# ChengZhang-98/lqer

Measured on AMD Instinct MI355X. Metric: W4A8+rank-r Linear GEMM TFLOPS-equiv, higher is better.
Workload: dtype bf16; 1 GPU; LqerLinear 4096x4096 rank32 W4A8-MXINT16 M=2048 (BASELINE configs[1]); rank=32, formats=x MXINT8/16, W MXINT4/16, A_out,B_out as x, y fp16, weights=one Linear

## Files before the change

include/lqer_hip.h:

```cpp
#ifndef LQER_HIP_H
#define LQER_HIP_H

#include <stddef.h>
#include <stdint.h>

#ifdef __cplusplus
extern "C" {
#endif

#define LQER_ABI_VERSION 14

#define LQER_OK 0
#define LQER_E_INVALID (-1)
#define LQER_E_UNSUPPORTED (-2)
#define LQER_E_LAUNCH (-3)
#define LQER_E_WORKSPACE (-4)

#define LQER_F32 0
#define LQER_F16 1
#define LQER_BF16 2

#define LQER_Q_PASSTHROUGH 0
#define LQER_Q_MXINT 1
#define LQER_Q_PASSTHROUGH_F16 2

#define LQER_Q_MXINT_I8 3

#define LQER_Q_INT 4

#define LQER_Q_MINIFLOAT 5

#define LQER_K_ALIGN 64
#define LQER_M_ALIGN 256
#define LQER_N_ALIGN 256
#define LQER_R_ALIGN 16
#define LQER_PANEL_ROWS 16
#define LQER_PANEL_BYTES 576

typedef struct lqer_qfmt {
  int32_t kind;
  int32_t width;
  int32_t block;
  int32_t exp_width;
  int32_t exp_bias;
} lqer_qfmt_t;

typedef struct lqer_linear_desc {
  int32_t in_features;
  int32_t out_features;
  int32_t rank;
  int32_t has_bias;
  lqer_qfmt_t x_fmt;
  lqer_qfmt_t w_fmt;
  lqer_qfmt_t b_fmt;
  lqer_qfmt_t a_out_fmt;
  lqer_qfmt_t b_out_fmt;
  int32_t tuning;
} lqer_linear_desc_t;

#define LQER_TUNE_TILE_ROWS_128 0x1
#define LQER_TUNE_TILE_ROWS_64 0x2
#define LQER_TUNE_I8_ROWS_128 0x4
#define LQER_TUNE_I8_ROWS_256 0x8
#define LQER_TUNE_AMAX_ATOMIC 0x40000
#define LQER_TUNE_AMAX_PARTS 0x80000
#define LQER_TUNE_AMAX_XCH_MISS 0x100000
#define LQER_TUNE_ACT8_SPLIT 0x200000
#define LQER_TUNE_ACT8_FUSED 0x400000
#define LQER_TUNE_ACT16_SPLIT 0x800000
#define LQER_TUNE_ACT16_FUSED 0x1000000
#define LQER_TUNE_AMAX_NO_MRX 0x4000000
#define LQER_TUNE_BOUT_IN_PROLOGUE 0x2000000
#define LQER_TUNE_DECODE_NO_POLL 0x10000

typedef struct lqer_linear_sizes {
  size_t w_packed;
  size_t a_t;
  size_t b_t;
  size_t bias_q;
  size_t workspace;
} lqer_linear_sizes_t;

int lqer_version(void);
const char* lqer_last_error(void);
size_t lqer_sizeof_qfmt(void);
size_t lqer_sizeof_linear_desc(void);
size_t lqer_sizeof_linear_sizes(void);
size_t lqer_sizeof_group_member(void);

int64_t lqer_padded_k(int64_t K);
int64_t lqer_padded_n(int64_t N);
int64_t lqer_padded_m(int64_t M);
int64_t lqer_padded_r(int64_t r);


int lqer_quantize_mxint(const void* x, int dtype, int64_t rows, int64_t cols, int64_t ld,
                        const lqer_qfmt_t* fmt, float* deq_f32, int8_t* codes, int8_t* exps,
                        void* stream);

int lqer_quantize_mxint_tiles(const void* x, int dtype, int64_t batches, int64_t rows, int64_t cols, const lqer_qfmt_t* fmt,
                              int64_t tile_rows, int64_t tile_cols, float* deq_f32, float* amax_scratch, void* stream);

int lqer_quantize_act_mxint(const void* x, int dtype, int64_t M, int64_t K, int64_t ldx,
                            const lqer_qfmt_t* fmt, void* xq_bf16, void* stream);


int lqer_linear_sizes(const lqer_linear_desc_t* desc, int64_t m_max, lqer_linear_sizes_t* out);

int lqer_pack_weight_mxint(const void* W, int dtype, int64_t N, int64_t K, int64_t ldw,
                           const lqer_qfmt_t* fmt, void* w_packed, void* scratch, void* stream);
int lqer_pack_weight_mxint_2d(const void* W, int dtype, int64_t N, int64_t K, int64_t ldw,
                              const lqer_qfmt_t* fmt, int64_t block_rows, void* w_packed, void* scratch,
                              void* stream);

int lqer_unpack_weight_mxint(const void* w_packed, int64_t N, int64_t K, const lqer_qfmt_t* fmt,
                             float* w_f32, void* stream);

int lqer_pack_lowrank(const void* A, const void* B, int dtype, int64_t K, int64_t N, int64_t r,
                      void* a_t, void* b_t, int32_t* limb_flags, void* stream);

int lqer_pack_bias(const void* bias, int dtype, int64_t N, const lqer_qfmt_t* fmt, float* bias_q,
                   void* stream);


int lqer_linear_forward(const lqer_linear_desc_t* desc, const void* x, int dtype, int64_t M,
                        int64_t ldx, const void* w_packed, const void* a_t, const void* b_t,
                        int a_limbs, int b_limbs, const float* bias_q, void* y, int64_t ldy,
                        void* workspace, size_t workspace_bytes, void* stream);


int lqer_quantize_act_xa(const lqer_linear_desc_t* desc, const void* x, int dtype, int64_t M,
                         int64_t ldx, const void* a_t, int a_limbs, void* xq_bf16, void* xaq_bf16,
                         void* scratch, size_t scratch_bytes, void* stream);
size_t lqer_lowrank_xa_scratch_bytes(const lqer_linear_desc_t* desc, int64_t m_max);
size_t lqer_act_image_bytes(const lqer_linear_desc_t* desc, int64_t m_max);
int lqer_lowrank_xa(const lqer_linear_desc_t* desc, const void* xq_bf16, int64_t M,
                    const void* a_t, int a_limbs, void* xaq_bf16, void* scratch,
                    size_t scratch_bytes, void* stream);
size_t lqer_linear_gemm_scratch_bytes(const lqer_linear_desc_t* desc, int64_t m_max);
int lqer_linear_gemm(const lqer_linear_desc_t* desc, const void* xq_bf16, int64_t M,
                     const void* w_packed, const void* xaq_bf16, const void* b_t, int b_limbs,
                     const float* bias_q, void* y, int dtype, int64_t ldy, void* scratch,
                     size_t scratch_bytes, void* stream);
int lqer_quantize_act_xa_prep(const lqer_linear_desc_t* desc, const void* x, int dtype, int64_t M,
                              int64_t ldx, const void* a_t, int a_limbs, void* xq_bf16, void* xaq_bf16,
                              void* scratch, size_t scratch_bytes, void* gemm_scratch, size_t* ready_bytes, void* stream);
int lqer_linear_gemm_prepared(const lqer_linear_desc_t* desc, const void* xq_bf16, int64_t M,
                              const void* w_packed, const void* xaq_bf16, const void* b_t, int b_limbs,
                              const float* bias_q, void* y, int dtype, int64_t ldy, void* scratch,
                              size_t scratch_bytes, size_t ready_bytes, void* stream);

#define LQER_ROUTE_SMALLM 0
#define LQER_ROUTE_TILE128 1
#define LQER_ROUTE_TILE256 2
#define LQER_ROUTE_I8 3
// ... 64 lines not shown
```

lqer_amd/_lib.py:

```python
from __future__ import annotations

import ctypes as C
import os
import subprocess
from typing import Optional

_HERE = os.path.dirname(os.path.abspath(__file__))
LIB_PATH = os.environ.get("LQER_AMD_LIB") or os.path.join(_HERE, "liblqer_hip.so")
BUILD_SCRIPT = os.path.join(_HERE, "csrc", "build.sh")

ABI_VERSION = 14
F32, F16, BF16 = 0, 1, 2
Q_PASSTHROUGH, Q_MXINT, Q_PASSTHROUGH_F16, Q_MXINT_I8, Q_INT, Q_MINIFLOAT = 0, 1, 2, 3, 4, 5
K_ALIGN, M_ALIGN, N_ALIGN, R_ALIGN = 64, 256, 256, 16
ROUTE_SMALLM, ROUTE_TILE128, ROUTE_TILE256, ROUTE_I8 = 0, 1, 2, 3
TUNE_TILE_ROWS_128, TUNE_TILE_ROWS_64, TUNE_DECODE_NO_POLL = 0x1, 0x2, 0x10000
TUNE_I8_ROWS_128, TUNE_I8_ROWS_256, TUNE_AMAX_ATOMIC, TUNE_AMAX_PARTS = 0x4, 0x8, 0x40000, 0x80000
TUNE_ACT16_SPLIT, TUNE_ACT16_FUSED = 0x800000, 0x1000000
TUNE_ACT8_SPLIT, TUNE_ACT8_FUSED = 0x200000, 0x400000
TUNE_AMAX_NO_MRX = 0x4000000
TUNE_BOUT_IN_PROLOGUE = 0x2000000
TUNE_AMAX_XCH_MISS = 0x100000


class QFmt(C.Structure):
    _fields_ = [("kind", C.c_int32), ("width", C.c_int32), ("block", C.c_int32), ("exp_width", C.c_int32), ("exp_bias", C.c_int32)]


class LinearDesc(C.Structure):
    _fields_ = [
        ("in_features", C.c_int32),
        ("out_features", C.c_int32),
        ("rank", C.c_int32),
        ("has_bias", C.c_int32),
        ("x_fmt", QFmt),
        ("w_fmt", QFmt),
        ("b_fmt", QFmt),
        ("a_out_fmt", QFmt),
        ("b_out_fmt", QFmt),
        ("tuning", C.c_int32),
    ]


class GroupMember(C.Structure):
    _fields_ = [("desc", C.POINTER(LinearDesc)), ("w_packed", C.c_void_p), ("b_t", C.c_void_p), ("b_limbs", C.c_int32),
                ("bias_q", C.c_void_p), ("y", C.c_void_p), ("ldy", C.c_int64)]


class LinearSizes(C.Structure):
    _fields_ = [("w_packed", C.c_size_t), ("a_t", C.c_size_t), ("b_t", C.c_size_t), ("bias_q", C.c_size_t), ("workspace", C.c_size_t)]


_vp, _i, _i64, _sz = C.c_void_p, C.c_int, C.c_int64, C.c_size_t
_qp, _dp = C.POINTER(QFmt), C.POINTER(LinearDesc)
_sp = C.POINTER(C.c_int64)

SIGNATURES = {
    "lqer_version": (_i, []),
    "lqer_last_error": (C.c_char_p, []),
    "lqer_sizeof_qfmt": (_sz, []),
    "lqer_sizeof_linear_desc": (_sz, []),
    "lqer_sizeof_linear_sizes": (_sz, []),
    "lqer_sizeof_group_member": (_sz, []),
    "lqer_padded_k": (_i64, [_i64]),
    "lqer_padded_n": (_i64, [_i64]),
    "lqer_padded_m": (_i64, [_i64]),
    "lqer_padded_r": (_i64, [_i64]),
    "lqer_quantize_mxint": (_i, [_vp, _i, _i64, _i64, _i64, _qp, _vp, _vp, _vp, _vp]),
    "lqer_quantize_mxint_tiles": (_i, [_vp, _i, _i64, _i64, _i64, _qp, _i64, _i64, _vp, _vp, _vp]),
    "lqer_quantize_act_mxint": (_i, [_vp, _i, _i64, _i64, _i64, _qp, _vp, _vp]),
    "lqer_linear_sizes": (_i, [_dp, _i64, C.POINTER(LinearSizes)]),
    "lqer_pack_weight_mxint": (_i, [_vp, _i, _i64, _i64, _i64, _qp, _vp, _vp, _vp]),
    "lqer_pack_weight_mxint_2d": (_i, [_vp, _i, _i64, _i64, _i64, _qp, _i64, _vp, _vp, _vp]),
    "lqer_unpack_weight_mxint": (_i, [_vp, _i64, _i64, _qp, _vp, _vp]),
    "lqer_pack_lowrank": (_i, [_vp, _vp, _i, _i64, _i64, _i64, _vp, _vp, _vp, _vp]),
    "lqer_pack_bias": (_i, [_vp, _i, _i64, _qp, _vp, _vp]),
    "lqer_linear_forward": (_i, [_dp, _vp, _i, _i64, _i64, _vp, _vp, _vp, _i, _i, _vp, _vp, _i64, _vp, _sz, _vp]),
    "lqer_quantize_act_xa": (_i, [_dp, _vp, _i, _i64, _i64, _vp, _i, _vp, _vp, _vp, _sz, _vp]),
    "lqer_lowrank_xa_scratch_bytes": (_sz, [_dp, _i64]),
    "lqer_act_image_bytes": (_sz, [_dp, _i64]),
    "lqer_lowrank_xa": (_i, [_dp, _vp, _i64, _vp, _i, _vp, _vp, _sz, _vp]),
    "lqer_linear_gemm_scratch_bytes": (_sz, [_dp, _i64]),
    "lqer_linear_gemm": (_i, [_dp, _vp, _i64, _vp, _vp, _vp, _i, _vp, _vp, _i, _i64, _vp, _sz, _vp]),
    "lqer_quantize_act_xa_prep": (_i, [_dp, _vp, _i, _i64, _i64, _vp, _i, _vp, _vp, _vp, _sz, _vp, C.POINTER(_sz), _vp]),
    "lqer_linear_gemm_prepared": (_i, [_dp, _vp, _i64, _vp, _vp, _vp, _i, _vp, _vp, _i, _i64, _vp, _sz, _sz, _vp]),
    "lqer_linear_gemm_ld": (_i, [_dp, _vp, _i64, _vp, _vp, _i64, _vp, _i, _vp, _vp, _i, _i64, _vp, _sz, _vp]),
    "lqer_desc_limbs": (_i, [_dp, C.POINTER(C.c_int), C.POINTER(C.c_int)]),
    "lqer_replicate_rows": (_i, [_vp, _vp, _i64, _i64, _i, _vp]),
    "lqer_decode_partials": (_i, [_dp, _i64]),
    "lqer_tile_partials": (_i, [_dp, _i64, _i]),
    "lqer_group_workspace_bytes": (_sz, [_i64, _i64]),
    "lqer_linear_forward_group": (_i, [C.POINTER(GroupMember), _i, _vp, _i, _i64, _i64, _vp, _i, _vp, _sz, _vp]),
    "lqer_gemm_route": (_i, [_dp, _i64, _i]),
    "lqer_gemm_tile_rows": (_i, [_dp, _i64, _i]),
    "lqer_f16_prepare": (_i, [_vp, _i64, _i64, _vp, _i, _i64, _vp, _vp, _vp]),
    "lqer_a_f16_image_bytes": (C.c_size_t, [_i64, _i64]),
    "lqer_a_b16_image_bytes": (C.c_size_t, [_i64, _i64]),
    "lqer_a_b16_prepare": (_i, [_vp, _i64, _i64, _vp, _vp]),
    "lqer_i8_prepare": (_i, [_vp, _i64, _i64, _qp, _vp, _vp]),
    "lqer_unpack_weight_i8": (_i, [_vp, _i64, _i64, _vp, _vp]),
    "lqer_unpack_weight_i8_fmt": (_i, [_vp, _i64, _i64, _qp, _vp, _vp]),
    "lqer_quantize_act_i8": (_i, [_vp, _i, _i64, _i64, _i64, _qp, _vp, _vp]),
    "lqer_clock_probe": (_i, [_vp, _i, _i64, _vp]),
    "lqer_col_abs_stats_workspace_bytes": (_sz, [_i64, _i64]),
# ... 47 lines not shown
```

lqer_amd/csrc/gemm_w4a8.hip:

```cpp
#include <atomic>
#include <type_traits>

#include "common.h"

namespace lqer {

constexpr int BM = 128, BN = 256, BK = 64;
#ifndef LQER_DEPTH
#define LQER_DEPTH 3
#endif
constexpr int DEPTH = LQER_DEPTH;
constexpr int NSLOT = DEPTH + 1;
constexpr int R_SLOT = (BN / 16) * LQER_PANEL_BYTES;
constexpr int OFF_A = 0;
constexpr int a_slot_bytes(int mt) { return 32 * mt * BK * 2; }
constexpr int gemm_lds_bytes(int mt) { return NSLOT * a_slot_bytes(mt) + NSLOT * R_SLOT; }

__device__ __forceinline__ int swz(int r, int c) { return r * 128 + ((c ^ ((r >> 1) & 7)) << 4); }

typedef __attribute__((address_space(3))) void lds_void;
typedef __attribute__((address_space(1))) const void gbl_void;

__device__ __forceinline__ float pair32_max(float v) {
  auto r = __builtin_amdgcn_permlane32_swap(__float_as_uint(v), __float_as_uint(v), false, false);
  return fmaxf(__uint_as_float(r[0]), __uint_as_float(r[1]));
}


template <int OFF>
__device__ __forceinline__ bf16x8 lds_read128(uint32_t addr) {
  bf16x8 v;
  asm volatile("ds_read_b128 %0, %1 offset:%2" : "=v"(v) : "v"(addr), "i"(OFF));
  return v;
}
__device__ __forceinline__ u32x4 lds_read128u(uint32_t addr) {
  u32x4 v;
  asm volatile("ds_read_b128 %0, %1" : "=v"(v) : "v"(addr));
  return v;
}
__device__ __forceinline__ uint32_t lds_read32_512(uint32_t addr) {
  uint32_t v;
  asm volatile("ds_read_b32 %0, %1 offset:512" : "=v"(v) : "v"(addr));
  return v;
}
__device__ __forceinline__ u32x2 lds_read64(uint32_t addr) {
  u32x2 v;
  asm volatile("ds_read_b64 %0, %1" : "=v"(v) : "v"(addr));
  return v;
}
__device__ __forceinline__ int lds_read_i8_512(uint32_t addr) {
  int v;
  asm volatile("ds_read_i8 %0, %1 offset:512" : "=v"(v) : "v"(addr));
  return v;
}
__device__ __forceinline__ void lds_write128(uint32_t addr, u32x4 v) {
  asm volatile("ds_write_b128 %0, %1" ::"v"(addr), "v"(v) : "memory");
}
__device__ __forceinline__ void lds_wait(bf16x8& a, bf16x8& b, bf16x8& c, bf16x8& d) {
  asm volatile("s_waitcnt lgkmcnt(0)" : "+v"(a), "+v"(b), "+v"(c), "+v"(d));
}
__device__ __forceinline__ void lds_wait(bf16x8& a, bf16x8& b) {
  asm volatile("s_waitcnt lgkmcnt(0)" : "+v"(a), "+v"(b));
}
__device__ __forceinline__ void lds_wait(u32x2& a, int& b) {
  asm volatile("s_waitcnt lgkmcnt(0)" : "+v"(a), "+v"(b));
}

#ifdef LQER_STAMPS
#define LQER_LOAD_BARRIER ""
#else
#define LQER_LOAD_BARRIER "\n\ts_barrier"
#endif
#if defined(LQER_STAMPS) || defined(LQER_CLOCKPROBE)
__device__ unsigned long long* g_stamp_buf = nullptr;
#endif
#ifdef LQER_STAMPS
#define STAMP(i)                                                                        \
  do {                                                                                  \
    unsigned long long t_;                                                              \
    __builtin_amdgcn_sched_barrier(0);                                                  \
    asm volatile("s_memtime %0\n\ts_waitcnt lgkmcnt(0)" : "=s"(t_)::"memory");         \
    __builtin_amdgcn_sched_barrier(0);                                                  \
    st_sum[i] += t_ - st_prev;                                                          \
    st_prev = t_;                                                                       \
  } while (0)
#else
#define STAMP(i)
#endif

template <int DT, bool LOWRANK, int BOUT, bool STAGED = false, int MT = 4, bool WTWOS = false, bool DEFER = false, bool WMF = false>
__global__ __launch_bounds__(512) void k_lqer_gemm(GemmArgs g) {
  static_assert(MT == 4 || MT == 2, "128- or 64-row tiles");
  static_assert(!DEFER || (LOWRANK && BOUT == 1 && MT == 4), "deferred B_out: blocks of 16 on 128-row tiles");
  static_assert(!WTWOS || DT != LQER_F16X, "integer weights: no fp16 main loop");
  constexpr int BMk = 32 * MT;
  constexpr int AP = MT / 2;
  constexpr bool XF16 = DT == LQER_F16X;
  constexpr int A_SLOT = a_slot_bytes(MT), OFF_R = NSLOT * A_SLOT;
  extern __shared__ __attribute__((aligned(16))) unsigned char smem[];
  const int tid = threadIdx.x, lane = tid & 63;
  const int wave = __builtin_amdgcn_readfirstlane(tid >> 6);
  const int wn = wave;
  const int l31 = lane & 31, lh = lane >> 5;
#ifdef LQER_CLOCKPROBE
  unsigned long long cp_rin, cp_rq = 0;
  asm volatile("s_memrealtime %0\n\ts_waitcnt lgkmcnt(0)" : "=s"(cp_rin)::"memory");
#endif

  const int nt = g.tiles_m * g.tiles_n;
  int tile;
  {
    const int b = blockIdx.x, xcd = b & 7, q8 = nt >> 3, r8 = nt & 7;
    tile = (xcd < r8 ? xcd * (q8 + 1) : r8 * (q8 + 1) + (xcd - r8) * q8) + (b >> 3);
  }
  const int tm = tile / g.tiles_n, tn = tile - tm * g.tiles_n;
  const int m0 = tm * BMk, n0 = tn * BN;
  const int nk = g.Kp / BK;

  const auto a_rsrc = __builtin_amdgcn_make_buffer_rsrc((void*)(g.xq + (int64_t)m0 * g.Kp), 0, BMk * g.Kp * 2, 0x00020000);
  int a_voff[2] = {0, 0};
#pragma unroll
  for (int i = 0; i < AP; ++i) {
    const int row = wave * (8 * AP) + i * 8 + (lane >> 3);
    const int chunk = (lane & 7) ^ ((row >> 1) & 7);
    a_voff[i] = (row * g.Kp + chunk * 8) * 2;
  }
  const uint8_t* w_base = g.wp + ((int64_t)(n0 / 16) * nk) * LQER_PANEL_BYTES;
  const auto w_rsrc = __builtin_amdgcn_make_buffer_rsrc((void*)w_base, 0, 16 * nk * LQER_PANEL_BYTES, 0x00020000);
  auto w_piece_voff = [&](int piece) {
    const int byte = piece * 1024 + lane * 16;
    const int pnl = byte / LQER_PANEL_BYTES;
    return pnl * nk * LQER_PANEL_BYTES + (byte - pnl * LQER_PANEL_BYTES);
  };
  const int w_voff = w_piece_voff(wave), w_voff8 = w_piece_voff(8);
  unsigned char* const a_dst0 = smem + OFF_A + wave * (8 * AP) * 128;
  unsigned char* const w_dst0 = smem + OFF_R + wave * 1024;
  auto issue_loads = [&](int kt, int slot) {
#pragma unroll
    for (int i = 0; i < AP; ++i)
      __builtin_amdgcn_raw_ptr_buffer_load_lds(a_rsrc, (lds_void*)(a_dst0 + slot * A_SLOT + i * 1024), 16, a_voff[i],
                                               kt * (BK * 2), 0, 0);
    __builtin_amdgcn_raw_ptr_buffer_load_lds(w_rsrc, (lds_void*)(w_dst0 + slot * R_SLOT), 16, w_voff, kt * LQER_PANEL_BYTES, 0, 0);
    if (wave == 0)
      __builtin_amdgcn_raw_ptr_buffer_load_lds(w_rsrc, (lds_void*)(smem + OFF_R + 8192 + slot * R_SLOT), 16, w_voff8,
                                               kt * LQER_PANEL_BYTES, 0, 0);
  };
  const uint32_t lds0 = (uint32_t)(uintptr_t)(lds_void*)smem;
  uint32_t fa_addr[4];
#pragma unroll
  for (int ks = 0; ks < 4; ++ks) fa_addr[ks] = lds0 + OFF_A + swz(l31, 2 * ks + lh);
  const int nw = wn * 32 + l31;
  const uint32_t fw_addr = lds0 + OFF_R + (nw >> 4) * LQER_PANEL_BYTES + (nw & 15) * 32 + lh * 16;
  const uint32_t fe_addr = lds0 + OFF_R + (nw >> 4) * LQER_PANEL_BYTES + (nw & 15) * 4;

  constexpr int STG = STAGED ? BMk * 8 / 512 : 1;
  u32x4 stg[STG];
  bf16x8 sb[STAGED ? 2 : 1][STAGED ? 4 : 1];
  const uint32_t stage = lds0 + OFF_A + (NSLOT - 1) * A_SLOT;
  const bf16_t* const bt_row = STAGED ? g.bt + (int64_t)(n0 + wn * 32 + l31) * g.rp + 8 * lh : nullptr;
  auto side_fetch_b = [&](int p0, int l, auto buf_c) {
    constexpr int BUF = decltype(buf_c)::value;
    if constexpr (STAGED) {
      const int cols = g.rp - p0 < 64 ? g.rp - p0 : 64;
#pragma unroll
      for (int ks = 0; ks < 4; ++ks)
        if (l < g.b_limbs && ks * 16 < cols) sb[BUF][ks] = *(const bf16x8*)(bt_row + (int64_t)l * g.Np * g.rp + p0 + ks * 16);
    }
  };
  auto side_fetch = [&](int p0) {
    if constexpr (!STAGED) return;
    const int cols = g.rp - p0 < 64 ? g.rp - p0 : 64;
    const int cpr = cols >> 3;
#pragma unroll
    for (int j = 0; j < STG; ++j) {
      const int c = tid + 512 * j;
      if (c < BMk * cpr) {
        const int row = c / cpr, ch = c - row * cpr;
        stg[j] = *(const u32x4*)(g.xaq + (int64_t)(m0 + row) * g.xaq_ld + p0 + 8 * ch);
      }
    }
    side_fetch_b(p0, 0, std::integral_constant<int, 0>{});
  };
  constexpr bool side_staged = LOWRANK && STAGED;
  if constexpr (side_staged) side_fetch(0);
  constexpr bool side_direct = LOWRANK && !STAGED;
  bf16x8 db[side_direct ? 2 : 1], dx[side_direct ? 2 : 1][side_direct ? MT : 1];
  const bool two_limbs = g.b_limbs > 1;
  if constexpr (side_direct) {
#pragma unroll
    for (int sl = 0; sl < 2; ++sl) {
      const int l = two_limbs ? sl : 0, ks = two_limbs ? 0 : sl;
// ... 200 lines not shown
    u32x4 wr;
    uint32_t we;
    if constexpr (MT == 4) {
      asm volatile(
          "ds_read_b128 %0, %18 offset:%c25\n\tds_read_b32 %1, %19 offset:%c25+512\n\t"
          "ds_read_b128 %2, %20 offset:%c24\n\tds_read_b128 %3, %20 offset:%c24+4096\n\t"
          "ds_read_b128 %4, %20 offset:%c24+8192\n\tds_read_b128 %5, %20 offset:%c24+12288\n\t"
          "ds_read_b128 %6, %21 offset:%c24\n\tds_read_b128 %7, %21 offset:%c24+4096\n\t"
          "ds_read_b128 %8, %21 offset:%c24+8192\n\tds_read_b128 %9, %21 offset:%c24+12288\n\t"
          "ds_read_b128 %10, %22 offset:%c24\n\tds_read_b128 %11, %22 offset:%c24+4096\n\t"
          "ds_read_b128 %12, %22 offset:%c24+8192\n\tds_read_b128 %13, %22 offset:%c24+12288\n\t"
          "ds_read_b128 %14, %23 offset:%c24\n\tds_read_b128 %15, %23 offset:%c24+4096\n\t"
          "ds_read_b128 %16, %23 offset:%c24+8192\n\tds_read_b128 %17, %23 offset:%c24+12288\n\t"
          "s_mov_b32 m0, %32\n\ts_nop 0\n\tbuffer_load_dwordx4 %26, %30, %36 offen lds\n\t"
          "s_mov_b32 m0, %33\n\ts_nop 0\n\tbuffer_load_dwordx4 %27, %30, %36 offen lds\n\t"
          "s_mov_b32 m0, %34\n\ts_nop 0\n\tbuffer_load_dwordx4 %28, %31, %37 offen lds\n\t"
          "s_cmp_lg_u32 %38, 0\n\ts_cbranch_scc1 1f\n\t"
          "s_mov_b32 m0, %35\n\ts_nop 0\n\tbuffer_load_dwordx4 %29, %31, %37 offen lds\n\t"
          "1:\n\ts_waitcnt vmcnt(6) lgkmcnt(0)"
          : "=&v"(wr), "=&v"(we), "=&v"(xa[0][0]), "=&v"(xa[0][1]), "=&v"(xa[0][2]), "=&v"(xa[0][3]), "=&v"(xa[1][0]),
            "=&v"(xa[1][1]), "=&v"(xa[1][2]), "=&v"(xa[1][3]), "=&v"(xa[2][0]), "=&v"(xa[2][1]), "=&v"(xa[2][2]),
            "=&v"(xa[2][3]), "=&v"(xa[3][0]), "=&v"(xa[3][1]), "=&v"(xa[3][2]), "=&v"(xa[3][3])
          : "v"(fw_addr), "v"(fe_addr), "v"(fa_addr[0]), "v"(fa_addr[1]), "v"(fa_addr[2]), "v"(fa_addr[3]),
            "i"(SLOT * A_SLOT), "i"(SLOT * R_SLOT),
            "v"(a_voff[0]), "v"(a_voff[1]), "v"(w_voff), "v"(w_voff8),
            "s"(a_rs), "s"(w_rs), "s"(m0a0), "s"(m0a1), "s"(m0w), "s"(m0w8), "s"(a_soff), "s"(w_soff), "s"(wave)
          : "memory", "scc");
    } else {
      asm volatile(
          "ds_read_b128 %0, %10 offset:%c17\n\tds_read_b32 %1, %11 offset:%c17+512\n\t"
          "ds_read_b128 %2, %12 offset:%c16\n\tds_read_b128 %3, %12 offset:%c16+4096\n\t"
          "ds_read_b128 %4, %13 offset:%c16\n\tds_read_b128 %5, %13 offset:%c16+4096\n\t"
          "ds_read_b128 %6, %14 offset:%c16\n\tds_read_b128 %7, %14 offset:%c16+4096\n\t"
          "ds_read_b128 %8, %15 offset:%c16\n\tds_read_b128 %9, %15 offset:%c16+4096\n\t"
          "s_mov_b32 m0, %23\n\ts_nop 0\n\tbuffer_load_dwordx4 %18, %21, %26 offen lds\n\t"
          "s_mov_b32 m0, %24\n\ts_nop 0\n\tbuffer_load_dwordx4 %19, %22, %27 offen lds\n\t"
          "s_cmp_lg_u32 %28, 0\n\ts_cbranch_scc1 1f\n\t"
          "s_mov_b32 m0, %25\n\ts_nop 0\n\tbuffer_load_dwordx4 %20, %22, %27 offen lds\n\t"
          "1:\n\ts_waitcnt vmcnt(4) lgkmcnt(0)"
          : "=&v"(wr), "=&v"(we), "=&v"(xa[0][0]), "=&v"(xa[0][1]), "=&v"(xa[1][0]), "=&v"(xa[1][1]), "=&v"(xa[2][0]),
            "=&v"(xa[2][1]), "=&v"(xa[3][0]), "=&v"(xa[3][1])
          : "v"(fw_addr), "v"(fe_addr), "v"(fa_addr[0]), "v"(fa_addr[1]), "v"(fa_addr[2]), "v"(fa_addr[3]),
            "i"(SLOT * A_SLOT), "i"(SLOT * R_SLOT),
            "v"(a_voff[0]), "v"(w_voff), "v"(w_voff8),
            "s"(a_rs), "s"(w_rs), "s"(m0a0), "s"(m0w), "s"(m0w8), "s"(a_soff), "s"(w_soff), "s"(wave)
          : "memory", "scc");
    }
    STAMP(1);
    auto expand = [&](uint32_t word, uint32_t scale_bits) {
      if constexpr (WMF) return expand_frag_lut(word, scale_bits, g.w_lut[0], g.w_lut[1]);
      else if constexpr (WTWOS) return expand_frag_twos(word, scale_bits);
      else return expand_frag_t<XF16>(word, scale_bits);
    };
    bf16x8 wb_first = expand(wr[0], (we & 0xffu) << 23);
    asm volatile("s_barrier" : "+v"(wb_first)::"memory");
    __builtin_amdgcn_s_setprio(0);
    __builtin_amdgcn_sched_barrier(0);
    STAMP(4);
    defer_piece(piece_c);
#pragma unroll
    for (int ks = 0; ks < 4; ++ks) {
      const uint32_t sc = ((we >> (8 * ks)) & 0xffu) << 23;
      const bf16x8 wb = ks == 0 ? wb_first : expand(wr[ks], sc);
#pragma unroll
      for (int i = 0; i < MT; ++i) acc[i] = mfma_32x32x16<XF16>(wb, xa[ks][i], acc[i]);
    }
    defer_pin(piece_c);
    __builtin_amdgcn_sched_barrier(0);
    STAMP(5);
    asm volatile("s_barrier" ::: "memory");
    __builtin_amdgcn_sched_barrier(0);
    STAMP(6);
  };
  using std::integral_constant;
  constexpr integral_constant<int, -1> no_piece{};
  int kt0 = 0;
  if constexpr (DEFER) {
#define LQER_DSTEP(KT) step(KT, integral_constant<int, (KT) % NSLOT>{}, integral_constant<int, KT>{})
    LQER_DSTEP(0); LQER_DSTEP(1); LQER_DSTEP(2); LQER_DSTEP(3); LQER_DSTEP(4); LQER_DSTEP(5); LQER_DSTEP(6); LQER_DSTEP(7);
    LQER_DSTEP(8); LQER_DSTEP(9); LQER_DSTEP(10); LQER_DSTEP(11); LQER_DSTEP(12); LQER_DSTEP(13); LQER_DSTEP(14); LQER_DSTEP(15);
#undef LQER_DSTEP
    kt0 = 16;
  }
  if (kt0 < nk)
  for (int kt = kt0;; kt += NSLOT) {
    step(kt, integral_constant<int, 0>{}, no_piece);
    if (kt + 1 >= nk) break;
    step(kt + 1, integral_constant<int, 1>{}, no_piece);
    if (kt + 2 >= nk) break;
    step(kt + 2, integral_constant<int, 2>{}, no_piece);
    if (kt + 3 >= nk) break;
    step(kt + 3, integral_constant<int, 3>{}, no_piece);
    if (kt + 4 >= nk) break;
  }
  asm volatile("s_waitcnt vmcnt(0)" ::: "memory");
  if (!late) asm volatile("s_barrier" ::: "memory");
#ifdef LQER_CLOCKPROBE
  {
    unsigned long long cp_c1, cp_r1;
    asm volatile("s_memtime %0\n\ts_memrealtime %1\n\ts_waitcnt lgkmcnt(0)" : "=s"(cp_c1), "=s"(cp_r1)::"memory");
    if (g_stamp_buf && lane == 0) {
      g_stamp_buf[(blockIdx.x * 8 + wave) * 8 + 0] = cp_c1 - cp_c0;
      g_stamp_buf[(blockIdx.x * 8 + wave) * 8 + 1] = cp_r1 - cp_r0;
      g_stamp_buf[(blockIdx.x * 8 + wave) * 8 + 2] = cp_rin;
      g_stamp_buf[(blockIdx.x * 8 + wave) * 8 + 3] = cp_r0;
      g_stamp_buf[(blockIdx.x * 8 + wave) * 8 + 4] = cp_r1;
      g_stamp_buf[(blockIdx.x * 8 + wave) * 8 + 7] = cp_rq;
    }
  }
#endif
#ifdef LQER_STAMPS
  if (g_stamp_buf && lane == 0)
    for (int i = 0; i < 8; ++i) g_stamp_buf[(blockIdx.x * 8 + wave) * 8 + i] = st_sum[i];
#endif

  if constexpr (DEFER) {
#pragma unroll
    for (int i = 0; i < MT; ++i)
#pragma unroll
      for (int k = 0; k < 16; ++k) acc[i][k] += sp[i][k];
  }
  const bool aligned16 = (((uintptr_t)g.y) & 15) == 0;
  const int nb = n0 + wn * 32;
#pragma unroll
  for (int i = 0; i < MT; ++i) {
    const int m = m0 + i * 32 + l31;
    if constexpr (DT == LQER_F32) {
#pragma unroll
      for (int q = 0; q < 4; ++q) {
        const int n = nb + 8 * q + 4 * lh;
        if (m < g.M) {
          float* dst = (float*)g.y + (int64_t)m * g.ldy + n;
          if (n + 3 < g.N && (g.ldy & 3) == 0 && aligned16) {
            *(float4*)dst = make_float4(acc[i][4 * q], acc[i][4 * q + 1], acc[i][4 * q + 2], acc[i][4 * q + 3]);
          } else {
#pragma unroll
            for (int t = 0; t < 4; ++t)
              if (n + t < g.N) dst[t] = acc[i][4 * q + t];
          }
        }
      }
    } else {
      uint32_t pk[4][2];
#pragma unroll
      for (int q = 0; q < 4; ++q)
#pragma unroll
        for (int h = 0; h < 2; ++h) {
          const float v0 = acc[i][4 * q + 2 * h], v1 = acc[i][4 * q + 2 * h + 1];
          if constexpr (DT == LQER_F16 || DT == LQER_F16X) {
            typedef __attribute__((ext_vector_type(2))) _Float16 h2;
            h2 hv = {(_Float16)v0, (_Float16)v1};
            pk[q][h] = __builtin_bit_cast(uint32_t, hv);
          } else {
            pk[q][h] = (uint32_t)f32_to_bf16_rne(v0) | ((uint32_t)f32_to_bf16_rne(v1) << 16);
          }
        }
      const bool wide = (g.ldy & 7) == 0 && nb + 32 <= g.N && aligned16;
#pragma unroll
      for (int p = 0; p < 2; ++p) {
        const uint32_t a0 = pk[2 * p][0], a1 = pk[2 * p][1], b0 = pk[2 * p + 1][0], b1 = pk[2 * p + 1][1];
        if (wide) {
          auto r0 = __builtin_amdgcn_permlane32_swap(a0, b0, false, false);
          auto r1 = __builtin_amdgcn_permlane32_swap(a1, b1, false, false);
          if (m < g.M) {
            bf16_t* dst = (bf16_t*)g.y + (int64_t)m * g.ldy + nb + 16 * p + 8 * lh;
            *(uint4*)dst = make_uint4(r0[0], r1[0], r0[1], r1[1]);
          }
        } else if (m < g.M) {
#pragma unroll
          for (int qq = 0; qq < 2; ++qq) {
            const int n = nb + 8 * (2 * p + qq) + 4 * lh;
            const uint32_t lo = qq ? b0 : a0, hi = qq ? b1 : a1;
            bf16_t* dst = (bf16_t*)g.y + (int64_t)m * g.ldy + n;
            if (n < g.N) dst[0] = (bf16_t)(lo & 0xffff);
            if (n + 1 < g.N) dst[1] = (bf16_t)(lo >> 16);
            if (n + 2 < g.N) dst[2] = (bf16_t)(hi & 0xffff);
            if (n + 3 < g.N) dst[3] = (bf16_t)(hi >> 16);
          }
        }
      }
    }
  }
#ifdef LQER_CLOCKPROBE
  {
    unsigned long long cp_r2, cp_r3;
    asm volatile("s_memrealtime %0\n\ts_waitcnt lgkmcnt(0)" : "=s"(cp_r2)::"memory");
    asm volatile("s_waitcnt vmcnt(0)\n\ts_memrealtime %0\n\ts_waitcnt lgkmcnt(0)" : "=s"(cp_r3)::"memory");
    if (g_stamp_buf && lane == 0) {
      g_stamp_buf[(blockIdx.x * 8 + wave) * 8 + 5] = cp_r2;
      g_stamp_buf[(blockIdx.x * 8 + wave) * 8 + 6] = cp_r3;
    }
  }
#endif
}

#ifndef LQER_AMAX_WAVES
#define LQER_AMAX_WAVES 2048
#endif
template <int RG, int NKS>
__global__ __launch_bounds__(256) void k_bout_amax(GemmArgs g, int tiles_n32, int seg_tiles) {
  const int lane = threadIdx.x & 63;
  const int64_t wid = (int64_t)blockIdx.x * 4 + (threadIdx.x >> 6);
  const int64_t groups = ((g.M + 31) / 32 + RG - 1) / RG;
  const int nseg = (tiles_n32 + seg_tiles - 1) / seg_tiles;
  if (wid >= groups * nseg) return;
  const int tg = (int)(wid / nseg), sg = (int)(wid - (int64_t)tg * nseg);
  const int l31 = lane & 31, lh = lane >> 5;
  const int Mp = (g.M + LQER_M_ALIGN - 1) / LQER_M_ALIGN * LQER_M_ALIGN;
  bf16x8 xa[RG][NKS];
  int rowv[RG];
#pragma unroll
  for (int u = 0; u < RG; ++u) {
    const int row = (tg * RG + u) * 32 + l31;
    rowv[u] = row < Mp ? row : -1;
    const int rc = row < Mp ? row : Mp - 1;
#pragma unroll
    for (int ks = 0; ks < NKS; ++ks) xa[u][ks] = *(const bf16x8*)(g.xaq + (int64_t)rc * g.xaq_ld + ks * 16 + 8 * lh);
  }
  const int t_begin = sg * seg_tiles;
  const int t_end = t_begin + seg_tiles < tiles_n32 ? t_begin + seg_tiles : tiles_n32;
  int cur_blk = (t_begin * 32) / g.bout_L;
  float cur[RG];
#pragma unroll
  for (int u = 0; u < RG; ++u) cur[u] = 0.f;
  auto commit = [&]() {
#pragma unroll
    for (int u = 0; u < RG; ++u) {
      const float m = pair32_max(cur[u]);
      if (lh == 0 && rowv[u] >= 0) {
        if (g.bout_nseg > 0) g.bout_amax[(int64_t)sg * Mp + rowv[u]] = m;
        else atomicMax((unsigned int*)g.bout_amax + (int64_t)rowv[u] * g.bout_nblk + cur_blk, __float_as_uint(m));
      }
    }
  };
  const f32x16 zero = {0, 0, 0, 0, 0, 0, 0, 0, 0, 0, 0, 0, 0, 0, 0, 0};
  const int nb = (t_end - t_begin) * g.b_limbs;
  const int64_t limb_stride = (int64_t)g.Np * g.rp;
  const bf16_t* const b_lane = g.bt + (int64_t)l31 * g.rp + 8 * lh;
  bf16x8 ba[NKS], bb[NKS];
  auto load = [&](int i, bf16x8 (&dst)[NKS]) {
    const int ii = i < nb ? i : nb - 1;
    const int tn = t_begin + ii / g.b_limbs, l = ii - (ii / g.b_limbs) * g.b_limbs;
    const bf16_t* p = b_lane + l * limb_stride + (int64_t)tn * 32 * g.rp;
#pragma unroll
    for (int ks = 0; ks < NKS; ++ks) dst[ks] = *(const bf16x8*)(p + ks * 16);
  };
  f32x16 acc[RG];
  int tn = t_begin, l = 0;
  auto consume = [&](const bf16x8 (&src)[NKS]) {
#pragma unroll
    for (int ks = 0; ks < NKS; ++ks) {
      if (l == 0 && ks == 0) {
#pragma unroll
        for (int u = 0; u < RG; ++u) acc[u] = __builtin_amdgcn_mfma_f32_32x32x16_bf16(src[0], xa[u][0], zero, 0, 0, 0);
      } else {
#pragma unroll
        for (int u = 0; u < RG; ++u) acc[u] = __builtin_amdgcn_mfma_f32_32x32x16_bf16(src[ks], xa[u][ks], acc[u], 0, 0, 0);
      }
    }
    if (++l == g.b_limbs) {
#pragma unroll
      for (int b = 0; b < 2; ++b) {
        const int blk = (tn * 32 + 16 * b) / g.bout_L;
        if (blk != cur_blk) {
          commit();
          cur_blk = blk;
#pragma unroll
          for (int u = 0; u < RG; ++u) cur[u] = 0.f;
        }
#pragma unroll
        for (int u = 0; u < RG; ++u) {
          float m = cur[u];
#pragma unroll
          for (int k = 0; k < 8; k += 2) m = fmaxf(fmaxf(m, fabsf(acc[u][8 * b + k])), fabsf(acc[u][8 * b + k + 1]));
          cur[u] = m;
        }
// ... 126 lines not shown
}

template <int DT>
static int launch_gemm(const GemmArgs& g, bool lowrank, int bout, hipStream_t st) {
  const unsigned grid = (unsigned)(g.tiles_m * g.tiles_n);
#define LQER_GEMM_LAUNCH(LR, BO)                                                                                \
  do {                                                                                                          \
    static LdsLimitOnce lds_once;                                                                               \
    lds_once.set((const void*)k_lqer_gemm<DT, LR, BO>, gemm_lds_bytes(4));                                      \
    k_lqer_gemm<DT, LR, BO><<<grid, 512, gemm_lds_bytes(4), st>>>(g);                                           \
  } while (0)
#define LQER_GEMM_LAUNCH_STAGED(BO)                                                                             \
  do {                                                                                                          \
    static LdsLimitOnce lds_once;                                                                               \
    lds_once.set((const void*)k_lqer_gemm<DT, true, BO, true>, gemm_lds_bytes(4));                              \
    k_lqer_gemm<DT, true, BO, true><<<grid, 512, gemm_lds_bytes(4), st>>>(g);                                   \
  } while (0)
#ifndef LQER_STAGE_MIN
#define LQER_STAGE_MIN 32
#endif
  const bool staged = lowrank && g.rp * g.b_limbs > LQER_STAGE_MIN;
  if (g.w_mf || bout == 3) {
    if constexpr (DT == LQER_F16X) {
      set_error("linear_gemm: minifloat weights and B_out have no fp16 main loop (pass-through fp16 activations take the limb route)");
      return LQER_E_UNSUPPORTED;
    } else {
#define LQER_GEMM_LAUNCH_MF(LR, BO, ST, WM)                                                                     \
  do {                                                                                                          \
    static LdsLimitOnce lds_once;                                                                               \
    lds_once.set((const void*)k_lqer_gemm<DT, LR, BO, ST, 4, false, false, WM>, gemm_lds_bytes(4));             \
    k_lqer_gemm<DT, LR, BO, ST, 4, false, false, WM><<<grid, 512, gemm_lds_bytes(4), st>>>(g);                  \
  } while (0)
      if (!g.w_mf) {
        if (g.w_twos) {
          static LdsLimitOnce lds_once;
          lds_once.set((const void*)k_lqer_gemm<DT, true, 3, true, 4, true>, gemm_lds_bytes(4));
          k_lqer_gemm<DT, true, 3, true, 4, true><<<grid, 512, gemm_lds_bytes(4), st>>>(g);
        } else if (staged) LQER_GEMM_LAUNCH_MF(true, 3, true, false);
        else LQER_GEMM_LAUNCH_MF(true, 3, false, false);
      } else if (!lowrank) LQER_GEMM_LAUNCH_MF(false, 0, false, true);
      else if (bout == 1) LQER_GEMM_LAUNCH_MF(true, 1, true, true);
      else if (bout == 2) LQER_GEMM_LAUNCH_MF(true, 2, true, true);
      else if (bout == 3) LQER_GEMM_LAUNCH_MF(true, 3, true, true);
      else LQER_GEMM_LAUNCH_MF(true, 0, true, true);
#undef LQER_GEMM_LAUNCH_MF
      return check_launch("lqer_gemm");
    }
  }
  if (g.w_twos) {
    if constexpr (DT == LQER_F16X) {
      set_error("linear_gemm: integer weights have no fp16 main loop (pass-through fp16 activations take the limb route)");
      return LQER_E_UNSUPPORTED;
    } else {
#define LQER_GEMM_LAUNCH_TWOS(LR, BO, ST)                                                                       \
  do {                                                                                                          \
    static LdsLimitOnce lds_once;                                                                               \
    lds_once.set((const void*)k_lqer_gemm<DT, LR, BO, ST, 4, true>, gemm_lds_bytes(4));                         \
    k_lqer_gemm<DT, LR, BO, ST, 4, true><<<grid, 512, gemm_lds_bytes(4), st>>>(g);                              \
  } while (0)
      if (!lowrank) LQER_GEMM_LAUNCH_TWOS(false, 0, false);
      else if (bout == 1) LQER_GEMM_LAUNCH_TWOS(true, 1, true);
      else if (bout == 2) LQER_GEMM_LAUNCH_TWOS(true, 2, true);
      else LQER_GEMM_LAUNCH_TWOS(true, 0, true);
#undef LQER_GEMM_LAUNCH_TWOS
      return check_launch("lqer_gemm");
    }
  }
#define LQER_GEMM_LAUNCH_H64(LR, BO, ST)                                                                        \
  do {                                                                                                          \
    static LdsLimitOnce lds_once;                                                                               \
    lds_once.set((const void*)k_lqer_gemm<DT, LR, BO, ST, 2>, gemm_lds_bytes(2));                               \
    k_lqer_gemm<DT, LR, BO, ST, 2><<<grid, 512, gemm_lds_bytes(2), st>>>(g);                                    \
  } while (0)
  if (g.tiles_m_rows == 64) {
    if (!lowrank) LQER_GEMM_LAUNCH_H64(false, 0, false);
    else if (bout == 1) { if (staged) LQER_GEMM_LAUNCH_H64(true, 1, true); else LQER_GEMM_LAUNCH_H64(true, 1, false); }
    else if (bout == 2) { if (staged) LQER_GEMM_LAUNCH_H64(true, 2, true); else LQER_GEMM_LAUNCH_H64(true, 2, false); }
    else { if (staged) LQER_GEMM_LAUNCH_H64(true, 0, true); else LQER_GEMM_LAUNCH_H64(true, 0, false); }
    return check_launch("lqer_gemm");
  }
#undef LQER_GEMM_LAUNCH_H64
  const bool defer = lowrank && bout == 1 && !(g.tuning & LQER_TUNE_BOUT_IN_PROLOGUE) && g.Kp / BK >= 16 && g.bout.kind == LQER_Q_MXINT &&
                     g.bout.mmax <= 4194304.0f && g.bout.mneg <= 4194304.0f && g.bout.tiny >= 1e-8f;
#define LQER_GEMM_LAUNCH_DEFER(ST)                                                                              \
  do {                                                                                                          \
    static LdsLimitOnce lds_once;                                                                               \
    lds_once.set((const void*)k_lqer_gemm<DT, true, 1, ST, 4, false, true>, gemm_lds_bytes(4));                 \
    k_lqer_gemm<DT, true, 1, ST, 4, false, true><<<grid, 512, gemm_lds_bytes(4), st>>>(g);                      \
  } while (0)
  if (!lowrank)
    LQER_GEMM_LAUNCH(false, 0);
  else if (bout == 1 && defer) {
    if (staged) LQER_GEMM_LAUNCH_DEFER(true); else LQER_GEMM_LAUNCH_DEFER(false);
  } else if (bout == 1) {
    if (staged) LQER_GEMM_LAUNCH_STAGED(1); else LQER_GEMM_LAUNCH(true, 1);
  } else if (bout == 2) {
    if (staged) LQER_GEMM_LAUNCH_STAGED(2); else LQER_GEMM_LAUNCH(true, 2);
  } else {
    if (staged) LQER_GEMM_LAUNCH_STAGED(0); else LQER_GEMM_LAUNCH(true, 0);
  }
#undef LQER_GEMM_LAUNCH_STAGED
#undef LQER_GEMM_LAUNCH
  return check_launch("lqer_gemm");
}

#if defined(LQER_STAMPS) || defined(LQER_CLOCKPROBE)
extern "C" int lqer_debug_set_stamp_buffer(void* p) {
  return (int)hipMemcpyToSymbol(HIP_SYMBOL(g_stamp_buf), &p, sizeof(p));
}
#endif

size_t gemm_scratch_bytes(int64_t m_max, int64_t N, const QP& bout) {
  if (bout.kind != LQER_Q_MXINT || bout.block == 16) return 0;
  const int64_t Np = lqer_padded_n(N);
  const int64_t L = (bout.block <= 0 || bout.block >= N) ? Np : bout.block;
  const int64_t nblk = (Np + L - 1) / L;
  return (size_t)lqer_padded_m(m_max) * (nblk == 1 ? 2 * LQER_AMAX_NSEG : nblk) * sizeof(float);
}

static int bout_mode(const GemmArgs& g, bool lowrank, int* L_out) {
  if (lowrank && g.bout.kind == LQER_Q_MXINT) {
    if (g.bout.block == 16) return 1;
    const int L = (g.bout.block <= 0 || g.bout.block >= g.N) ? g.Np : g.bout.block;
    if (L % 16 != 0) {
      set_error("B_out_quantizer block %d: must be a multiple of 16 or cover the row", g.bout.block);
      return LQER_E_UNSUPPORTED;
    }
    if (L_out) *L_out = L;
    return 2;
  }
  if (lowrank && g.bout.kind == LQER_Q_INT) {
    if (L_out) *L_out = 0;
    return 2;
  }
  if (lowrank && g.bout.kind == LQER_Q_MINIFLOAT) {
    if (L_out) *L_out = 0;
    return 3;
  }
  if (lowrank && g.bout.kind != LQER_Q_PASSTHROUGH) {
    set_error("B_out_quantizer kind %d not implemented", g.bout.kind);
    return LQER_E_UNSUPPORTED;
  }
  return 0;
}

int gemm_route(const GemmArgs& g, bool lowrank) {
  const int bout = bout_mode(g, lowrank, nullptr);
  if (bout < 0) return bout;
  if (g.w8) {
    GemmArgs t = g;
    if (bout == 2 && g.bout.kind == LQER_Q_MXINT) {
      const int L = (g.bout.block <= 0 || g.bout.block >= g.N) ? g.Np : g.bout.block;
      t.bout_nblk = (g.Np + L - 1) / L;
    }
    if (i8_eligible(t, bout)) return LQER_ROUTE_I8;
    t.w8 = nullptr;
    return gemm_route(t, lowrank);
  }
  if (g.w_twos) return LQER_ROUTE_TILE128;
  if (g.w_mf || bout == 3) return LQER_ROUTE_TILE128;
  if (smallm_eligible(g, bout)) return LQER_ROUTE_SMALLM;
  if (m256_eligible(g)) return LQER_ROUTE_TILE256;
  return LQER_ROUTE_TILE128;
}

int gemm_tile_rows(const GemmArgs& g) {
  constexpr int CUS = 256;
  const int64_t tn = g.Np / BN;
  const int64_t t128 = (int64_t)((g.M + BM - 1) / BM) * tn, t64 = (int64_t)((g.M + 63) / 64) * tn;
  const int pin = (g.tuning & LQER_TUNE_TILE_ROWS_128) ? 128 : ((g.tuning & LQER_TUNE_TILE_ROWS_64) ? 64 : 0);
  const bool mf = g.w_mf || g.bout.kind == LQER_Q_MINIFLOAT;
  if (!g.w_twos && !mf && ((pin != 128 && 2 * t128 <= CUS && t64 > t128 && g.M > 64) || (pin == 64 && g.M > 64))) return 64;
  return BM;
}

__global__ void k_zero_cells(uint32_t* p, int64_t n) {
// ... 151 lines not shown
```

Baseline: 1069 TFLOP/s-equiv.

## Overlap output stores with the last k-step in deferred B_out GEMM

Adds a TAIL instantiation of the deferred-B_out GEMM kernel that peels the final k-step out of the main loop. It interleaves the MFMAs of that step with packing and buffer-storing finished accumulator rows, so the epilogue store latency hides under the remaining compute. A new tuning flag can disable the path, and a fallback handles unaligned or edge tiles. The cost is more instruction-scheduling complexity and register pressure, plus a dependence on the ring-slot and LDS offset assumptions.

Measured after the change: 1068 TFLOP/s-equiv. Within noise of the previous version (-0.1%).

```diff
diff --git a/include/lqer_hip.h b/include/lqer_hip.h
--- a/include/lqer_hip.h
+++ b/include/lqer_hip.h
@@ -71,6 +71,7 @@
 #define LQER_TUNE_ACT16_FUSED 0x1000000
 #define LQER_TUNE_AMAX_NO_MRX 0x4000000
 #define LQER_TUNE_BOUT_IN_PROLOGUE 0x2000000
+#define LQER_TUNE_TAIL_BEHIND_LOOP 0x8000000
 #define LQER_TUNE_DECODE_NO_POLL 0x10000
 
 typedef struct lqer_linear_sizes {
diff --git a/lqer_amd/_lib.py b/lqer_amd/_lib.py
--- a/lqer_amd/_lib.py
+++ b/lqer_amd/_lib.py
@@ -20,6 +20,7 @@
 TUNE_ACT8_SPLIT, TUNE_ACT8_FUSED = 0x200000, 0x400000
 TUNE_AMAX_NO_MRX = 0x4000000
 TUNE_BOUT_IN_PROLOGUE = 0x2000000
+TUNE_TAIL_BEHIND_LOOP = 0x8000000
 TUNE_AMAX_XCH_MISS = 0x100000
 
 
diff --git a/lqer_amd/csrc/gemm_w4a8.hip b/lqer_amd/csrc/gemm_w4a8.hip
--- a/lqer_amd/csrc/gemm_w4a8.hip
+++ b/lqer_amd/csrc/gemm_w4a8.hip
@@ -88,10 +88,11 @@
 #define STAMP(i)
 #endif
 
-template <int DT, bool LOWRANK, int BOUT, bool STAGED = false, int MT = 4, bool WTWOS = false, bool DEFER = false, bool WMF = false>
+template <int DT, bool LOWRANK, int BOUT, bool STAGED = false, int MT = 4, bool WTWOS = false, bool DEFER = false, bool WMF = false, bool TAIL = false>
 __global__ __launch_bounds__(512) void k_lqer_gemm(GemmArgs g) {
   static_assert(MT == 4 || MT == 2, "128- or 64-row tiles");
   static_assert(!DEFER || (LOWRANK && BOUT == 1 && MT == 4), "deferred B_out: blocks of 16 on 128-row tiles");
+  static_assert(!TAIL || (DEFER && !WTWOS && !WMF), "stores under the last k-step: the deferred-B_out instantiations");
   static_assert(!WTWOS || DT != LQER_F16X, "integer weights: no fp16 main loop");
   constexpr int BMk = 32 * MT;
   constexpr int AP = MT / 2;
@@ -107,6 +108,12 @@
   asm volatile("s_memrealtime %0\n\ts_waitcnt lgkmcnt(0)" : "=s"(cp_rin)::"memory");
 #endif
 
+#ifndef LQER_CLOCKPROBE
+  if constexpr (TAIL) {
+    asm volatile("" ::"s"(g.xq), "s"(g.wp), "s"(g.xaq), "s"(g.xaq_ld), "s"(g.bt), "s"(g.bias), "s"(g.y), "s"(g.ldy), "s"(g.M), "s"(g.N), "s"(g.Kp),
+                 "s"(g.rp), "s"(g.b_limbs), "s"(g.tiles_m), "s"(g.tiles_n));
+  }
+#endif
   const int nt = g.tiles_m * g.tiles_n;
   int tile;
   {
@@ -473,19 +480,19 @@
 #undef LQER_DSTEP
     kt0 = 16;
   }
-  if (kt0 < nk)
+  const int nk_loop = TAIL ? nk - 1 : nk;
+  if (kt0 < nk_loop)
   for (int kt = kt0;; kt += NSLOT) {
     step(kt, integral_constant<int, 0>{}, no_piece);
-    if (kt + 1 >= nk) break;
+    if (kt + 1 >= nk_loop) break;
     step(kt + 1, integral_constant<int, 1>{}, no_piece);
-    if (kt + 2 >= nk) break;
+    if (kt + 2 >= nk_loop) break;
     step(kt + 2, integral_constant<int, 2>{}, no_piece);
-    if (kt + 3 >= nk) break;
+    if (kt + 3 >= nk_loop) break;
     step(kt + 3, integral_constant<int, 3>{}, no_piece);
-    if (kt + 4 >= nk) break;
-  }
-  asm volatile("s_waitcnt vmcnt(0)" ::: "memory");
-  if (!late) asm volatile("s_barrier" ::: "memory");
+    if (kt + 4 >= nk_loop) break;
+  }
+  auto probe_loop_end = [&]() {
 #ifdef LQER_CLOCKPROBE
   {
     unsigned long long cp_c1, cp_r1;
@@ -504,6 +511,128 @@
   if (g_stamp_buf && lane == 0)
     for (int i = 0; i < 8; ++i) g_stamp_buf[(blockIdx.x * 8 + wave) * 8 + i] = st_sum[i];
 #endif
+  };
+  auto probe_stores = [&]() {
+#ifdef LQER_CLOCKPROBE
+    unsigned long long cp_r2, cp_r3;
+    asm volatile("s_memrealtime %0\n\ts_waitcnt lgkmcnt(0)" : "=s"(cp_r2)::"memory");
+    asm volatile("s_waitcnt vmcnt(0)\n\ts_memrealtime %0\n\ts_waitcnt lgkmcnt(0)" : "=s"(cp_r3)::"memory");
+    if (g_stamp_buf && lane == 0) {
+      g_stamp_buf[(blockIdx.x * 8 + wave) * 8 + 5] = cp_r2;
+      g_stamp_buf[(blockIdx.x * 8 + wave) * 8 + 6] = cp_r3;
+    }
+#endif
+  };
+  if constexpr (TAIL) {
+    constexpr int ES = DT == LQER_F32 ? 4 : 2;
+    constexpr int PPT = DT == LQER_F32 ? 4 : 2;
+    static_assert(NSLOT == 4, "ring of four slots");
+    const int nb = n0 + wn * 32;
+    const bool tail_stored = __builtin_amdgcn_readfirstlane((int)((g.ldy & (16 / ES - 1)) == 0 && nb + 32 <= g.N && (((uintptr_t)g.y) & 15) == 0)) != 0;
+    const int slot = __builtin_amdgcn_readfirstlane((nk - 1) & (NSLOT - 1));
+    const uint32_t ao = slot * A_SLOT, ro = slot * R_SLOT;
+    const uint32_t la0 = fa_addr[0] + ao, la1 = fa_addr[1] + ao, la2 = fa_addr[2] + ao, la3 = fa_addr[3] + ao;
+    const uint32_t lw = fw_addr + ro, le = fe_addr + ro;
+    STAMP(7);
+    __builtin_amdgcn_s_setprio(1);
+    bf16x8 xa[4][MT];
+    u32x4 wr;
+    uint32_t we;
+    asm volatile(
+        "ds_read_b128 %0, %10\n\tds_read_b32 %1, %11 offset:512\n\t"
+        "ds_read_b128 %2, %12\n\tds_read_b128 %3, %12 offset:4096\n\t"
+        "ds_read_b128 %4, %13\n\tds_read_b128 %5, %13 offset:4096\n\t"
+        "ds_read_b128 %6, %14\n\tds_read_b128 %7, %14 offset:4096\n\t"
+        "ds_read_b128 %8, %15\n\tds_read_b128 %9, %15 offset:4096\n\t"
+        "s_waitcnt vmcnt(0) lgkmcnt(0)"
+        : "=&v"(wr), "=&v"(we), "=&v"(xa[0][0]), "=&v"(xa[0][1]), "=&v"(xa[1][0]), "=&v"(xa[1][1]), "=&v"(xa[2][0]), "=&v"(xa[2][1]),
+          "=&v"(xa[3][0]), "=&v"(xa[3][1])
+        : "v"(lw), "v"(le), "v"(la0), "v"(la1), "v"(la2), "v"(la3)
+        : "memory");
+    STAMP(1);
+    bf16x8 wb[4];
+#pragma unroll
+    for (int ks = 0; ks < 4; ++ks) wb[ks] = expand_frag_t<XF16>(wr[ks], ((we >> (8 * ks)) & 0xffu) << 23);
+    asm volatile("s_barrier" : "+v"(wb[0]), "+v"(wb[1]), "+v"(wb[2]), "+v"(wb[3])::"memory");
+    __builtin_amdgcn_s_setprio(0);
+    __builtin_amdgcn_sched_barrier(0);
+    STAMP(4);
+    const auto y_rsrc = __builtin_amdgcn_make_buffer_rsrc(g.y, 0, (int)(g.M * g.ldy * ES), 0x00020000);
+    const int ldy = (int)g.ldy;
+    const int y_voff = ((m0 + l31) * ldy + nb + (16 / ES) * lh) * ES;
+    auto tail_part = [&](int i, int p) {
+      u32x4 out;
+      if constexpr (DT == LQER_F32) {
+#pragma unroll
+        for (int t = 0; t < 4; ++t) out[t] = __float_as_uint(acc[i][4 * p + t] + sp[i][4 * p + t]);
+      } else {
+        uint32_t pk[2][2];
+#pragma unroll
+        for (int qq = 0; qq < 2; ++qq)
+#pragma unroll
+          for (int h = 0; h < 2; ++h) {
+            const int k = 4 * (2 * p + qq) + 2 * h;
+            const float v0 = acc[i][k] + sp[i][k], v1 = acc[i][k + 1] + sp[i][k + 1];
+            if constexpr (DT == LQER_F16 || DT == LQER_F16X) {
+              typedef __attribute__((ext_vector_type(2))) _Float16 h2;
+              h2 hv = {(_Float16)v0, (_Float16)v1};
+              pk[qq][h] = __builtin_bit_cast(uint32_t, hv);
+            } else {
+              pk[qq][h] = (uint32_t)f32_to_bf16_rne(v0) | ((uint32_t)f32_to_bf16_rne(v1) << 16);
+            }
+          }
+        auto r0 = __builtin_amdgcn_permlane32_swap(pk[0][0], pk[1][0], false, false);
+        auto r1 = __builtin_amdgcn_permlane32_swap(pk[0][1], pk[1][1], false, false);
+        out = (u32x4){r0[0], r1[0], r0[1], r1[1]};
+      }
+      __builtin_amdgcn_raw_buffer_store_b128(out, y_rsrc, y_voff + (i * 32 * ldy + (32 / PPT) * p) * ES, 0, 0);
+    };
+    auto tail_compute = [&](auto stored_c) {
+      constexpr bool STORED = decltype(stored_c)::value;
+#pragma unroll
+      for (int j = 0; j < 16; ++j) {
+        if (j == 8) lds_wait(xa[0][2], xa[1][2], xa[2][2], xa[3][2]);
+        if (j == 12) lds_wait(xa[0][3], xa[1][3], xa[2][3], xa[3][3]);
+        acc[j >> 2] = mfma_32x32x16<XF16>(wb[j & 3], xa[j & 3][j >> 2], acc[j >> 2]);
+        if (j == 3) xa[0][2] = lds_read128<8192>(la0), xa[1][2] = lds_read128<8192>(la1), xa[2][2] = lds_read128<8192>(la2), xa[3][2] = lds_read128<8192>(la3);
+        if (j == 8) xa[0][3] = lds_read128<12288>(la0), xa[1][3] = lds_read128<12288>(la1), xa[2][3] = lds_read128<12288>(la2), xa[3][3] = lds_read128<12288>(la3);
+        if constexpr (STORED) {
+          if constexpr (DT != LQER_F32) __builtin_amdgcn_sched_barrier(0);
+#pragma unroll
+          for (int e = 0; e < 3 * PPT; ++e) {
+            const int at = 4 * (e / PPT) + 5 + (e % PPT) * (4 / PPT);
+            if ((at > 15 ? 15 : at) == j) tail_part(e / PPT, e % PPT);
+          }
+        }
+        __builtin_amdgcn_sched_barrier(0);
+      }
+      if constexpr (STORED) {
+#pragma unroll
+        for (int p = 0; p < PPT; ++p) tail_part(3, p);
+      }
+    };
+    if (tail_stored) {
+      tail_compute(std::true_type{});
+      __builtin_amdgcn_sched_barrier(0);
+      STAMP(5);
+      asm volatile("s_barrier" ::: "memory");
+      __builtin_amdgcn_sched_barrier(0);
+      STAMP(6);
+      if (!late) asm volatile("s_barrier" ::: "memory");
+      probe_loop_end();
+      probe_stores();
+      __builtin_amdgcn_endpgm();
+    }
+    tail_compute(std::false_type{});
+    __builtin_amdgcn_sched_barrier(0);
+    STAMP(5);
+    asm volatile("s_barrier" ::: "memory");
+    __builtin_amdgcn_sched_barrier(0);
+    STAMP(6);
+  }
+  if constexpr (!TAIL) asm volatile("s_waitcnt vmcnt(0)" ::: "memory");
+  if (!late) asm volatile("s_barrier" ::: "memory");
+  probe_loop_end();
 
   if constexpr (DEFER) {
 #pragma unroll
@@ -572,17 +701,7 @@
       }
     }
   }
-#ifdef LQER_CLOCKPROBE
-  {
-    unsigned long long cp_r2, cp_r3;
-    asm volatile("s_memrealtime %0\n\ts_waitcnt lgkmcnt(0)" : "=s"(cp_r2)::"memory");
-    asm volatile("s_waitcnt vmcnt(0)\n\ts_memrealtime %0\n\ts_waitcnt lgkmcnt(0)" : "=s"(cp_r3)::"memory");
-    if (g_stamp_buf && lane == 0) {
-      g_stamp_buf[(blockIdx.x * 8 + wave) * 8 + 5] = cp_r2;
-      g_stamp_buf[(blockIdx.x * 8 + wave) * 8 + 6] = cp_r3;
-    }
-  }
-#endif
+  probe_stores();
 }
 
 #ifndef LQER_AMAX_WAVES
@@ -875,16 +994,20 @@
 #undef LQER_GEMM_LAUNCH_H64
   const bool defer = lowrank && bout == 1 && !(g.tuning & LQER_TUNE_BOUT_IN_PROLOGUE) && g.Kp / BK >= 16 && g.bout.kind == LQER_Q_MXINT &&
                      g.bout.mmax <= 4194304.0f && g.bout.mneg <= 4194304.0f && g.bout.tiny >= 1e-8f;
-#define LQER_GEMM_LAUNCH_DEFER(ST)                                                                              \
+  const bool tail = defer && !(g.tuning & LQER_TUNE_TAIL_BEHIND_LOOP) && g.Kp / BK >= 17 && g.ldy > 0 &&
+                    ((int64_t)g.tiles_m * BM + 1) * g.ldy * 4 <= 0x7fffffffll;
+#define LQER_GEMM_LAUNCH_DEFER(ST, TL)                                                                          \
   do {                                                                                                          \
     static LdsLimitOnce lds_once;                                                                               \
-    lds_once.set((const void*)k_lqer_gemm<DT, true, 1, ST, 4, false, true>, gemm_lds_bytes(4));                 \
-    k_lqer_gemm<DT, true, 1, ST, 4, false, true><<<grid, 512, gemm_lds_bytes(4), st>>>(g);                      \
+    lds_once.set((const void*)k_lqer_gemm<DT, true, 1, ST, 4, false, true, false, TL>, gemm_lds_bytes(4));      \
+    k_lqer_gemm<DT, true, 1, ST, 4, false, true, false, TL><<<grid, 512, gemm_lds_bytes(4), st>>>(g);           \
   } while (0)
   if (!lowrank)
     LQER_GEMM_LAUNCH(false, 0);
-  else if (bout == 1 && defer) {
-    if (staged) LQER_GEMM_LAUNCH_DEFER(true); else LQER_GEMM_LAUNCH_DEFER(false);
+  else if (bout == 1 && defer && tail) {
+    if (staged) LQER_GEMM_LAUNCH_DEFER(true, true); else LQER_GEMM_LAUNCH_DEFER(false, true);
+  } else if (bout == 1 && defer) {
+    if (staged) LQER_GEMM_LAUNCH_DEFER(true, false); else LQER_GEMM_LAUNCH_DEFER(false, false);
   } else if (bout == 1) {
     if (staged) LQER_GEMM_LAUNCH_STAGED(1); else LQER_GEMM_LAUNCH(true, 1);
   } else if (bout == 2) {
```
